# AlexGeControl/Visual-Inertial-Odometry

Measured on AMD Instinct MI355X. Metric: GN iterations/s, 11-frame (10-keyframe) window, 20k landmarks per GPU, higher is better.
Workload: dtype f64

## Files before the change

visual-inertial-odometry_amd/csrc/vio_imu_math.h:

```cpp
#ifndef VIO_IMU_MATH_H
#define VIO_IMU_MATH_H

#pragma clang fp contract(off)

#include "vio_device_math.h"
#include "vio_types.h"

#define O_P 0
#define O_R 3
#define O_V 6
#define O_BA 9
#define O_BG 12

#pragma clang fp contract(off)
__device__ __forceinline__ void nc_quat_to_R(const double *q, double *R) {
    const double x = q[0], y = q[1], z = q[2], w = q[3];
    const double tx = 2 * x, ty = 2 * y, tz = 2 * z;
    const double twx = tx * w, twy = ty * w, twz = tz * w;
    const double txx = tx * x, txy = ty * x, txz = tz * x;
    const double tyy = ty * y, tyz = tz * y, tzz = tz * z;
    R[0] = 1 - (tyy + tzz); R[1] = txy - twz;       R[2] = txz + twy;
    R[3] = txy + twz;       R[4] = 1 - (txx + tzz); R[5] = tyz - twx;
    R[6] = txz - twy;       R[7] = tyz + twx;       R[8] = 1 - (txx + tyy);
}
__device__ __forceinline__ void nc_m3_mul(const double *A, const double *B, double *C) {
#pragma unroll
    for (int i = 0; i < 3; ++i)
#pragma unroll
        for (int j = 0; j < 3; ++j)
            C[3 * i + j] = A[3 * i] * B[j] + A[3 * i + 1] * B[3 + j] + A[3 * i + 2] * B[6 + j];
}
__device__ __forceinline__ dquat nc_qmul(dquat a, dquat b) {
    dquat r;
    r.w = a.w * b.w - a.x * b.x - a.y * b.y - a.z * b.z;
    r.x = a.w * b.x + a.x * b.w + a.y * b.z - a.z * b.y;
    r.y = a.w * b.y + a.y * b.w + a.z * b.x - a.x * b.z;
    r.z = a.w * b.z + a.z * b.w + a.x * b.y - a.y * b.x;
    return r;
}
__device__ __forceinline__ dquat nc_qinv(dquat q) {
    const double n2 = q.x * q.x + q.y * q.y + q.z * q.z + q.w * q.w;
    dquat r = {0, 0, 0, 0};
    if (n2 > 0) { r.x = -q.x / n2; r.y = -q.y / n2; r.z = -q.z / n2; r.w = q.w / n2; }
    return r;
}
__device__ __forceinline__ void nc_qrot(dquat q, const double *v, double *o) {
    double ux = q.y * v[2] - q.z * v[1], uy = q.z * v[0] - q.x * v[2], uz = q.x * v[1] - q.y * v[0];
    ux += ux; uy += uy; uz += uz;
    o[0] = v[0] + q.w * ux + (q.y * uz - q.z * uy);
    o[1] = v[1] + q.w * uy + (q.z * ux - q.x * uz);
    o[2] = v[2] + q.w * uz + (q.x * uy - q.y * ux);
}
struct ImuCommon {
    dquat Qi, Qj, Qi_inv, dq, cdq;
    double sum_dt;
    double dba[3], dbg[3];
};

__device__ __forceinline__ void d_qleft_br(dquat q, double *B) {
    double v[3] = {q.x, q.y, q.z};
    d_skew(v, B);
    B[0] += q.w; B[4] += q.w; B[8] += q.w;
}
__device__ __forceinline__ void d_qright_br(dquat q, double *B) {
    double v[3] = {q.x, q.y, q.z}, S[9];
    d_skew(v, S);
#pragma unroll
    for (int k = 0; k < 9; ++k) B[k] = -S[k];
    B[0] += q.w; B[4] += q.w; B[8] += q.w;
}

__device__ void d_imu_common(const double *pre, const double *pi, const double *si, const double *pj, ImuCommon &c) {
    c.Qi = d_qload(pi); c.Qj = d_qload(pj);
    c.Qi_inv = nc_qinv(c.Qi);
    c.sum_dt = pre[PRE_SUMDT];
    c.dq.x = pre[PRE_DQ]; c.dq.y = pre[PRE_DQ + 1]; c.dq.z = pre[PRE_DQ + 2]; c.dq.w = pre[PRE_DQ + 3];
#pragma unroll
    for (int k = 0; k < 3; ++k) { c.dba[k] = si[3 + k] - pre[PRE_BA + k]; c.dbg[k] = si[6 + k] - pre[PRE_BG + k]; }
    const double *Jm = pre + PRE_JAC;
    double th[3];
#pragma unroll
    for (int i = 0; i < 3; ++i)
        th[i] = Jm[15 * (O_R + i) + O_BG] * c.dbg[0] + Jm[15 * (O_R + i) + O_BG + 1] * c.dbg[1] + Jm[15 * (O_R + i) + O_BG + 2] * c.dbg[2];
    dquat dth = {th[0] / 2.0, th[1] / 2.0, th[2] / 2.0, 1.0};
    c.cdq = nc_qmul(c.dq, dth);
}

__device__ void d_imu_residual(const double *pre, const double *G, const double *pi, const double *si, const double *pj,
                               const double *sj, const ImuCommon &c, double *res) {
    const double *Jm = pre + PRE_JAC;
    const double sum_dt = c.sum_dt;
    double cdp[3], cdv[3];
#pragma unroll
    for (int i = 0; i < 3; ++i) {
        double a = 0, b = 0, e = 0, f = 0;
#pragma unroll
        for (int j = 0; j < 3; ++j) {
            a += Jm[15 * (O_V + i) + O_BA + j] * c.dba[j];
            b += Jm[15 * (O_V + i) + O_BG + j] * c.dbg[j];
            e += Jm[15 * (O_P + i) + O_BA + j] * c.dba[j];
            f += Jm[15 * (O_P + i) + O_BG + j] * c.dbg[j];
        }
        cdv[i] = pre[PRE_DV + i] + a + b;
        cdp[i] = pre[PRE_DP + i] + e + f;
    }
    double t[3], u[3];
#pragma unroll
    for (int k = 0; k < 3; ++k) t[k] = 0.5 * G[k] * sum_dt * sum_dt + pj[k] - pi[k] - si[k] * sum_dt;
    nc_qrot(c.Qi_inv, t, u);
#pragma unroll
    for (int k = 0; k < 3; ++k) res[O_P + k] = u[k] - cdp[k];
    dquat qe = nc_qmul(nc_qinv(c.cdq), nc_qmul(c.Qi_inv, c.Qj));
    res[O_R] = 2 * qe.x; res[O_R + 1] = 2 * qe.y; res[O_R + 2] = 2 * qe.z;
#pragma unroll
    for (int k = 0; k < 3; ++k) t[k] = G[k] * sum_dt + sj[k] - si[k];
    nc_qrot(c.Qi_inv, t, u);
#pragma unroll
    for (int k = 0; k < 3; ++k) res[O_V + k] = u[k] - cdv[k];
#pragma unroll
    for (int k = 0; k < 3; ++k) { res[O_BA + k] = sj[3 + k] - si[3 + k]; res[O_BG + k] = sj[6 + k] - si[6 + k]; }
}

__device__ __forceinline__ void d_imu_rit(const ImuCommon &c, double *RiT) {
    double qi[4] = {c.Qi_inv.x, c.Qi_inv.y, c.Qi_inv.z, c.Qi_inv.w};
    nc_quat_to_R(qi, RiT);
}
__device__ void d_imu_jac_block(int blk, const double *pre, const double *G, const double *pi, const double *si,
                                const double *pj, const double *sj, const ImuCommon &c, const double *RiT, double *sJ) {
    const double *Jm = pre + PRE_JAC;
    const double sum_dt = c.sum_dt;
    double B[9];
    int r0 = 0, c0 = 0;
    switch (blk) {
    case 0: r0 = O_P; c0 = 0 + O_P;
        for (int k = 0; k < 9; ++k) B[k] = -RiT[k];
        break;
    case 1: { r0 = O_P; c0 = 0 + O_R;
        double t[3], u[3];
        for (int k = 0; k < 3; ++k) t[k] = 0.5 * G[k] * sum_dt * sum_dt + pj[k] - pi[k] - si[k] * sum_dt;
        nc_qrot(c.Qi_inv, t, u); d_skew(u, B);
        break; }
    case 2: { r0 = O_R; c0 = 0 + O_R;
        dquat a = nc_qmul(nc_qinv(c.Qj), c.Qi), b = c.cdq;
        double La[9], Rb[9], P[9];
        d_qleft_br(a, La); d_qright_br(b, Rb); nc_m3_mul(La, Rb, P);
        const double va[3] = {a.x, a.y, a.z}, vb[3] = {b.x, b.y, b.z};
        for (int i = 0; i < 3; ++i) for (int j = 0; j < 3; ++j) B[3 * i + j] = -(va[i] * (-vb[j]) + P[3 * i + j]);
        break; }
    case 3: { r0 = O_V; c0 = 0 + O_R;
        double t[3], u[3];
        for (int k = 0; k < 3; ++k) t[k] = G[k] * sum_dt + sj[k] - si[k];
        nc_qrot(c.Qi_inv, t, u); d_skew(u, B);
        break; }
    case 4: r0 = O_P; c0 = 6 + 0;
        for (int k = 0; k < 9; ++k) B[k] = -RiT[k] * sum_dt;
        break;
    case 5: r0 = O_P; c0 = 6 + 3;
        for (int i = 0; i < 3; ++i) for (int j = 0; j < 3; ++j) B[3 * i + j] = -Jm[15 * (O_P + i) + O_BA + j];
        break;
    case 6: r0 = O_P; c0 = 6 + 6;
        for (int i = 0; i < 3; ++i) for (int j = 0; j < 3; ++j) B[3 * i + j] = -Jm[15 * (O_P + i) + O_BG + j];
        break;
    case 7: { r0 = O_R; c0 = 6 + 6;
        double L[9], nL[9], D[9];
        d_qleft_br(nc_qmul(nc_qmul(nc_qinv(c.Qj), c.Qi), c.dq), L);
        for (int k = 0; k < 9; ++k) nL[k] = -L[k];
        for (int i = 0; i < 3; ++i) for (int j = 0; j < 3; ++j) D[3 * i + j] = Jm[15 * (O_R + i) + O_BG + j];
        nc_m3_mul(nL, D, B);
        break; }
    case 8: r0 = O_V; c0 = 6 + 0;
        for (int k = 0; k < 9; ++k) B[k] = -RiT[k];
        break;
    case 9: r0 = O_V; c0 = 6 + 3;
        for (int i = 0; i < 3; ++i) for (int j = 0; j < 3; ++j) B[3 * i + j] = -Jm[15 * (O_V + i) + O_BA + j];
        break;
    case 10: r0 = O_V; c0 = 6 + 6;
        for (int i = 0; i < 3; ++i) for (int j = 0; j < 3; ++j) B[3 * i + j] = -Jm[15 * (O_V + i) + O_BG + j];
        break;
    case 11: r0 = O_P; c0 = 15 + O_P;
        for (int k = 0; k < 9; ++k) B[k] = RiT[k];
        break;
    case 12: { r0 = O_R; c0 = 15 + O_R;
        d_qleft_br(nc_qmul(nc_qmul(nc_qinv(c.cdq), c.Qi_inv), c.Qj), B);
        break; }
    case 13: r0 = O_V; c0 = 21 + 0;
        for (int k = 0; k < 9; ++k) B[k] = RiT[k];
        break;
    default: return;
    }
    for (int i = 0; i < 3; ++i) for (int j = 0; j < 3; ++j) sJ[30 * (r0 + i) + c0 + j] = B[3 * i + j];
}

#pragma clang fp contract(fast)

#endif
```

visual-inertial-odometry_amd/csrc/vio_pose_solve_chain.h:

```cpp
#ifndef VIO_POSE_SOLVE_CHAIN_H
#define VIO_POSE_SOLVE_CHAIN_H

#define CH_NS 11
#define CH_TS 11
#define CH_SCSZ (16 * CH_TS)
#define CH_S9SZ (9 * CH_TS)
#define CH_OFF_SC 0
#define CH_OFF_SO (CH_OFF_SC + CH_NS * 5 * CH_SCSZ)
#define CH_OFF_SD (CH_OFF_SO + 10 * CH_S9SZ)
#define CH_OFF_CC (CH_OFF_SD + CH_NS * CH_S9SZ)
#define CH_OFF_Y (CH_OFF_CC + 15 * PS_TS)
#define CH_YC 176
#define CH_NDIM 256
#define CH_PACKED ((CH_OFF_Y + CH_NDIM + 1) & ~1)
#define CH_SET_STRIDE 16128
#define CH_OFF_SM CH_PACKED
#define CH_OFF_MC (CH_OFF_SM + CH_NS * CH_S9SZ)
#define CH_OFF_D (CH_OFF_MC + PS_TS)
#define CH_OFF_X (CH_OFF_D + CH_NDIM)
#define CH_OFF_I9 (CH_OFF_X + CH_NDIM)
#define CH_OFF_I16 (CH_OFF_I9 + CH_S9SZ)
#define CH_OFF_NZ (CH_OFF_I16 + PS_TS)
#define CH_LDS_CORE (CH_OFF_NZ + 32)
static_assert(CH_NS * CH_S9SZ >= CH_NS * 64, "the back-substitution's scratch (11 x 64) lives in the SD tiles");
// ... 370 lines not shown
#pragma unroll
                for (int k = 0; k < 3; ++k) if (lane + 64 * k < STATE_STRIDE) sState[lane + 64 * k] = st[k];
                if (test_here) {
                    double w[3];
#pragma unroll
                    for (int k = 0; k < 3; ++k) w[k] = d_wave_sum_to_lane63(er[k] * er[k]);
                    const int valid = d_imu_mask(T);
                    double t_imu = 0.0;
#pragma unroll
                    for (int k = 0; k < 10; ++k) { const double c = d_readlane(ichi, k); if ((valid >> k) & 1) t_imu += c; }
                    if (lane == 63) {
                        double total = tv[0] + t_imu;
                        if (T.has_prior) total += sqrt((w[0] + w[1]) + w[2]);
                        const double tempChi = 0.5 * total;
                        const double scale = 0.5 * (tv[1] + ((tv[3] + tv[4]) + tv[5])) + 1e-6;
                        lm->chi_try = tempChi;
                        lm->scale = scale;
                        lm->rho = (tv[2] - tempChi) / scale;
                        lm->trials += 1;
                        lm->chi = tempChi;
                        lm->cur = cur;
                        lm->accepted = 1;
                        lm->naccepted += 1;
                        lm->need_linearize = 1;
                        lm->false_cnt = 0;
                        if (!isfinite(tempChi)) lm->finite = 0;
                    }
                }
            }
        }
    } else {
    if (SPLIT) {
        xs0 = cfi[CH_OFF_SM + tid];
        if (tid < CH_NS * CH_S9SZ - PS_THREADS) xs1 = cfi[CH_OFF_SM + PS_THREADS + tid];
        if (tid < CH_YC) { xd = cfi[CH_OFF_D + tid]; xy = cfi[CH_OFF_Y + tid]; }
        if (tid < 2) xe = cfi[CH_OFF_NZ + tid];
    }
    for (int pass = 0; pass < 2; ++pass) {
        const double2 *src = reinterpret_cast<const double2 *>(T.Pg + set * CH_SET_STRIDE);
        const double2 *csrc = reinterpret_cast<const double2 *>(cfi);
        double2 *dst = reinterpret_cast<double2 *>(P);
        static_assert((CH_PACKED / 2 + PS_THREADS - 1) / PS_THREADS == 8, "copy below is written for 8 rounds");
        static_assert(CH_OFF_SD % 2 == 0, "the range that comes from cfi is whole double2s");
#define CH_FROM_CFI(i2) (SPLIT && (i2) < CH_OFF_SD / 2)
#define CH_LD(q) const double2 v##q = (CH_FROM_CFI(tid + q * PS_THREADS) ? csrc : src)[min(tid + q * PS_THREADS, CH_PACKED / 2 - 1)];
#define CH_ST(q) dst[min(tid + q * PS_THREADS, CH_PACKED / 2 - 1)] = v##q;
        CH_LD(0) CH_LD(1) CH_LD(2) CH_LD(3) CH_LD(4) CH_LD(5) CH_LD(6) CH_LD(7)
        if (pass == 0) {
            double stv = (tid < STATE_STRIDE) ? T.state[cur * STATE_STRIDE + tid] : 0.0;
            const double stv1 = (lm_loop && tid < STATE_STRIDE) ? T.state[STATE_STRIDE + tid] : 0.0;
            const bool test_here = d_step_owed(T, VIO_GN_TEST_PREV);
            double t_chi = 0.0, t_step = 0.0, t_lmchi = 0.0, t_imu = 0.0, t_sp = 0.0;
            if (test_here) {
                const int lc = lm_loop ? (lm->cur ^ lm->pending) : cur;
                double e2 = 0.0;
                if (T.has_prior && tid < VIO_PRD) { const double er = T.errprior[lc * VIO_PRD_PAD + tid]; e2 = er * er; }
                if (tid < 192) { const double w = d_wave_sum_to_lane63(e2); if (lane == 63) sB[tid >> 6] = w; }
                if (uwave == 0) {
                    const int valid = d_imu_mask(T);
                    const double ichi = T.imu_out[min(lane, 9) * IMU_OUT + IMU_CHI];
                    t_chi = T.vis[VIS_CHI]; t_step = T.vis[VIS_STEP + 1]; t_lmchi = lm->chi;
                    t_sp = (T.sp_part[0] + T.sp_part[1]) + T.sp_part[2];
#pragma unroll
                    for (int k = 0; k < 10; ++k) { const double c = d_readlane(ichi, k); if ((valid >> k) & 1) t_imu += c; }
                }
            }
            int pend0 = 0, sys0 = 0;
            if (lm_loop && tid == 0 && test_here) { d_lm_load(lm, sLm); pend0 = lm->pending; sys0 = lm->sys; }
            if (lm_loop && tid == 0 && !test_here) {
                int go = 1, rej = 0, sys = lm->sys;
                d_lm_load(lm, sLm);
                if (lm->pending) {
                    d_lm_verdict(sLm, lm, 0, lm->chi_try, lm->scale, sLm.cur);
                    if (sLm.accepted) sys ^= 1; else rej = 1;
                    go = !sLm.stop;
                }
                sX[0] = go ? 1.0 : 0.0; sX[1] = (double)sLm.cur; sX[2] = sLm.lambda; sX[3] = (double)sys; sX[4] = (double)rej;
            }
            CH_ST(0) CH_ST(1) CH_ST(2) CH_ST(3) CH_ST(4) CH_ST(5) CH_ST(6) CH_ST(7)
            __syncthreads();
            if (test_here) {
                if (tid == 0) {
                    double total = t_chi + t_imu;
                    if (T.has_prior) total += sqrt((sB[0] + sB[1]) + sB[2]);
                    const double tempChi = 0.5 * total;
                    const double scale = 0.5 * (t_step + t_sp) + 1e-6;
                    lm->chi_try = tempChi;
                    lm->scale = scale;
                    if (!lm_loop) {
                        lm->rho = (t_lmchi - tempChi) / scale;
                        lm->trials += 1;
                        lm->chi = tempChi;
                        lm->cur = cur;
                        lm->accepted = 1;
                        lm->naccepted += 1;
                        lm->need_linearize = 1;
                        lm->false_cnt = 0;
                        if (!isfinite(tempChi)) lm->finite = 0;
                    } else {
                        int go = 1, rej = 0, sys = sys0;
                        if (pend0) {
                            d_lm_verdict(sLm, lm, 0, tempChi, scale, sLm.cur);
                            if (sLm.accepted) sys ^= 1; else rej = 1;
                            go = !sLm.stop;
                        }
                        sX[0] = go ? 1.0 : 0.0; sX[1] = (double)sLm.cur; sX[2] = sLm.lambda; sX[3] = (double)sys; sX[4] = (double)rej;
                    }
                }
                if (lm_loop) __syncthreads();
            }
            int set_now = 0;
            if (lm_loop) {
                if (tid == 0) { d_lm_store(lm, sLm); lm->sys = (int)sX[3]; lm->pending = sX[0] != 0.0 ? 1 : 0; }
                if (sX[0] == 0.0) return;
                cur = (int)sX[1]; lambda = sX[2]; set_now = (int)sX[3];
                if (cur) stv = stv1;
            }
            if (tid < STATE_STRIDE) sState[tid] = stv;
            if (set_now == set) break;
            set = set_now;
            __syncthreads();
        } else {
            CH_ST(0) CH_ST(1) CH_ST(2) CH_ST(3) CH_ST(4) CH_ST(5) CH_ST(6) CH_ST(7)
            __syncthreads();
        }
#undef CH_LD
#undef CH_ST
#undef CH_FROM_CFI
    }
    if (tid < n) {
        const int d = ch_dim(tid);
        if (d >= CH_YC) P[ch_cc_elem(d - CH_YC, d - CH_YC)] += lambda;
        else if (!SPLIT) P[ch_sd(d >> 4) + (d & 15) * (CH_TS + 1)] += lambda;
    } else if (tid < n + 8) {
        P[ch_cc_elem(72 + tid - n, 72 + tid - n)] = 1.0;
    } else if (tid >= 256 && tid < 256 + CH_S9SZ + PS_TS) {
        const int i = tid - 256;
        P[CH_OFF_I9 + i] = (i < CH_S9SZ) ? ((i / CH_TS == i % CH_TS) ? 1.0 : 0.0) : (((i - CH_S9SZ) / PS_TROW == (i - CH_S9SZ) % PS_TROW) ? 1.0 : 0.0);
    } else if (tid >= 640 && tid < 640 + CH_NDIM) {
        if (!SPLIT || tid - 640 >= CH_YC) P[CH_OFF_D + tid - 640] = 1.0;
    }
    if (SPLIT) {
        P[CH_OFF_SM + tid] = xs0;
        if (tid < CH_NS * CH_S9SZ - PS_THREADS) P[CH_OFF_SM + PS_THREADS + tid] = xs1;
        if (tid < CH_YC) { P[CH_OFF_D + tid] = xd; P[CH_OFF_Y + tid] = xy; }
        if (tid < 2) P[CH_OFF_NZ + tid] = xe;
    } else {
        for (int i = tid; i < CH_NS * CH_S9SZ; i += PS_THREADS) P[CH_OFF_SM + i] = 0.0;
    }
    __syncthreads();
    }
    CH_OUT(0);
    const int trial = cur ^ 1;
    const bool prior_here = T.has_prior && !(T.gn_flags & VIO_GN_PRIOR_LATER);
    const int lm_dim = T.lm_dim;
    double *pairtab_trial = T.pairtab + trial * PAIRTAB_STRIDE;
    double *pw = P + CH_OFF_CC;
    auto mid1 = [&](int ln) {
        if (prior_here || CH_DIAG_SKIP == 2) return;
        if (ln < 12) {
            const double *p = (ln == 0) ? sState + STATE_EXT : sState + STATE_POSE + 7 * (ln - 1);
            const double *d = (ln == 0) ? sX + CH_YC + 66 : sX + CH_YC + 6 * (ln - 1);
            double dd[6], tmp[7];
#pragma unroll
            for (int k = 0; k < 6; ++k) dd[k] = d[k];
            d_pose_plus(p, dd, tmp);
            double *q = (ln == 0) ? pw + STATE_EXT : pw + STATE_POSE + 7 * (ln - 1);
#pragma unroll
            for (int k = 0; k < 7; ++k) q[k] = tmp[k];
        }
        __builtin_amdgcn_wave_barrier();
        asm volatile("" ::: "memory");
        if (lm_dim != 3) d_pair_rotations(pw, pw + 96, ln);
    };
    auto mid2 = [&](int idx, int ln) {
        if (prior_here || lm_dim == 3 || CH_DIAG_SKIP == 1 || CH_DIAG_SKIP == 2) return;
        d_pair_rows(pw, pairtab_trial, pw + 96, ln + 64 * idx, 14 * 64);
    };
    const bool ext_trivial = T.ext_fixed && !T.marg_mode;
    if (SPLIT) {
        unsigned long long t0__ = 0ull;
#ifdef VIO_STAMPS
        t0__ = __builtin_amdgcn_s_memtime();
        if (tid == 0) { g_ch_dbg = T.dbg; g_ch_t0 = t0__; }
#endif
        const unsigned lo = (unsigned)P[CH_OFF_NZ], hi = (unsigned)P[CH_OFF_NZ + 1];
        const unsigned long long eff = ((unsigned long long)__builtin_amdgcn_readfirstlane(hi) << 32) | (unsigned long long)(unsigned)__builtin_amdgcn_readfirstlane(lo);
        ch_camera_solve<true>(P, tid, ch_lane(lane), eff, mid1, mid2, T.dbg, t0__, ext_trivial);
    } else {
        ch_factor_solve(P, tid, mid1, mid2, T.dbg, ext_trivial, early);
    }
    CH_OUT(2);
    for (int i = tid; i < n; i += PS_THREADS) sDx[i] = sX[ch_dim(i)];
    if (tid >= 192 && tid < 384 && T.sp_part) {
        const int i = tid - 192;
        const double dxi = (i < n) ? sX[ch_dim(min(i, n - 1))] : 0.0;
        const double bi = early ? bf_early : ((i < n) ? T.bfull[set * VIO_PD_PAD + i] : 0.0);
        const double w = d_wave_sum_to_lane63((i < n) ? dxi * (lambda * dxi + bi) : 0.0);
        if (lane == 63) T.sp_part[i >> 6] = w;
    }
    if (!prior_here) {
        if (tid >= 128 && tid < 128 + 84) sState[tid - 128] = P[CH_OFF_CC + tid - 128];
        else if (tid >= 256 && tid < 256 + 99) { const int e = tid - 256; sState[STATE_SB + e] += sX[(e / 9) * 16 + (e % 9 < 3 ? 6 + e % 9 : (e % 9 < 6 ? e % 9 : e % 9 - 6))]; }
        d_lds_barrier();
        if (tid >= 192 && tid < 192 + n) T.dx[tid - 192] = sDx[tid - 192];
        if (tid >= 384 && tid < 384 + STATE_STRIDE) T.state[trial * STATE_STRIDE + (tid - 384)] = sState[tid - 384];
        CH_OUT(3);
        return;
    }
    __syncthreads();

    if (uwave < 2) {
        if (tid < 12) {
            double *p = (tid == 0) ? sState + STATE_EXT : sState + STATE_POSE + 7 * (tid - 1);
            const double *d = (tid == 0) ? sDx : sDx + 6 + 15 * (tid - 1);
            double tmp[7];
            d_pose_plus(p, d, tmp);
            for (int k = 0; k < 7; ++k) p[k] = tmp[k];
        } else if (tid >= 16 && tid < 16 + 99) {
            const int e = tid - 16, f = e / 9, k = e % 9;
            sState[STATE_SB + e] = sState[STATE_SB + e] + sDx[12 + 15 * f + k];
        }
        __syncthreads();
        if (T.lm_dim != 3) d_pair_rotations(sState, sR, tid);
        __syncthreads();
    } else {
        {
            double hp[PS_PRIOR_ROWS][3], bp[PS_PRIOR_ROWS];
#pragma unroll
            for (int r = 0; r < PS_PRIOR_ROWS; ++r) {
                const int i = (uwave - 2) + 14 * r;
#pragma unroll
                for (int q = 0; q < 3; ++q) {
                    const int j = lane + 64 * q;
                    hp[r][q] = (i < n && j < n) ? T.Hprior[i * n + j] : 0.0;
                }
                bp[r] = (i < n) ? T.bprior[cur * VIO_PD_PAD + i] : 0.0;
            }
            const double x0 = sDx[lane], x1 = sDx[lane + 64], x2 = (lane + 128 < n) ? sDx[lane + 128] : 0.0;
#pragma unroll
            for (int r = 0; r < PS_PRIOR_ROWS; ++r) {
                const int i = (uwave - 2) + 14 * r;
                const double v = d_bprior_dot(hp[r][0], hp[r][1], hp[r][2], x0, x1, x2, bp[r]);
                if (lane == 63 && i < n) { sB[i] = v; T.bprior[trial * VIO_PD_PAD + i] = v; }
            }
        }
        __syncthreads();
        double jp[PS_JT_ROWS][3];
#pragma unroll
        for (int r = 0; r < PS_JT_ROWS; ++r) {
            const int i = (uwave - 2) + 14 * r;
#pragma unroll
            for (int q = 0; q < 3; ++q) {
                const int j = lane + 64 * q;
                jp[r][q] = (i < VIO_PRD && j < VIO_PRD) ? T.Jtinv[i * VIO_PRD + j] : 0.0;
            }
        }
        __syncthreads();
        {
            const double y0 = sB[lane], y1 = sB[lane + 64], y2 = (lane + 128 < VIO_PRD) ? sB[lane + 128] : 0.0;
#pragma unroll
            for (int r = 0; r < PS_JT_ROWS; ++r) {
                const int i = (uwave - 2) + 14 * r;
                const double s = d_errprior_dot(jp[r][0], jp[r][1], jp[r][2], y0, y1, y2);
                if (lane == 63 && i < VIO_PRD) T.errprior[trial * VIO_PRD_PAD + i] = s;
            }
        }
    }
    if (T.lm_dim != 3) d_pair_rows(sState, T.pairtab + trial * PAIRTAB_STRIDE, sR, tid, PS_THREADS);
    if (tid >= 192 && tid < 192 + n) T.dx[tid - 192] = sDx[tid - 192];
    if (tid >= 384 && tid < 384 + STATE_STRIDE) T.state[trial * STATE_STRIDE + (tid - 384)] = sState[tid - 384];
    CH_OUT(3);
}
__global__ __launch_bounds__(PS_THREADS) void k_pose_solve_c(DeviceTables T) { d_pose_solve_chain_body<false>(T); }
__global__ __launch_bounds__(PS_THREADS) void k_pose_solve_cb(BatchArgs a) { const DeviceTables T = d_batch_tables(a); d_pose_solve_chain_body<false>(T); }
__global__ __launch_bounds__(PS_THREADS) void k_pose_solve_cs(DeviceTables T) { d_pose_solve_chain_body<true>(T); }

__device__ __forceinline__ void ch_chain_pre_store(const double *P, int tid, unsigned long long eff, double *cfi) {
    {
        const double2 *s2 = reinterpret_cast<const double2 *>(P);
        double2 *d2 = reinterpret_cast<double2 *>(cfi);
        constexpr int N2 = CH_OFF_SD / 2;
        static_assert(5 * PS_THREADS < N2 && N2 <= 6 * PS_THREADS, "six rounds");
        const double2 v0 = s2[tid], v1 = s2[tid + PS_THREADS], v2 = s2[tid + 2 * PS_THREADS], v3 = s2[tid + 3 * PS_THREADS], v4 = s2[tid + 4 * PS_THREADS];
        const int i5 = tid + 5 * PS_THREADS;
        double2 v5 = make_double2(0.0, 0.0);
        if (i5 < N2) v5 = s2[i5];
        d2[tid] = v0; d2[tid + PS_THREADS] = v1; d2[tid + 2 * PS_THREADS] = v2; d2[tid + 3 * PS_THREADS] = v3; d2[tid + 4 * PS_THREADS] = v4;
        if (i5 < N2) d2[i5] = v5;
    }
    for (int i = tid; i < CH_NS * CH_S9SZ; i += PS_THREADS) cfi[CH_OFF_SM + i] = P[CH_OFF_SM + i];
    if (tid < CH_YC) { cfi[CH_OFF_D + tid] = P[CH_OFF_D + tid]; cfi[CH_OFF_Y + tid] = P[CH_OFF_Y + tid]; }
    if (tid == 0) { cfi[CH_OFF_NZ] = (double)(unsigned)(eff & 0xffffffffull); cfi[CH_OFF_NZ + 1] = (double)(unsigned)(eff >> 32); }
}
__device__ __forceinline__ void ch_chain_pre_init(double *P, int tid) {
    if (tid >= 256 && tid < 256 + CH_S9SZ) { const int i = tid - 256; P[CH_OFF_I9 + i] = (i / CH_TS == i % CH_TS) ? 1.0 : 0.0; }
    else if (tid >= 640 && tid < 640 + CH_YC) P[CH_OFF_D + tid - 640] = 1.0;
    for (int i = tid; i < CH_NS * CH_S9SZ; i += PS_THREADS) P[CH_OFF_SM + i] = 0.0;
}
#define CPI_PRE 0
#define CPI_J (CPI_PRE + 10 * PRE_STRIDE)
#define CPI_ST (CPI_J + 10 * 450)
#define CPI_CM (CPI_ST + 184)
#define CPI_JTI(k) ((k) < 9 ? CH_OFF_CC + 450 * (k) : CH_LDS_CORE)
#define CPI_VEC (CH_LDS_CORE + 450)
#define CPI_BP (CPI_VEC + 640)
#define CPI_PN (CPI_BP + VIO_PD_PAD)
#define CPI_END (CPI_PN + 2)
#define CPI_NTILES (55 + 10 + 11)
#define CPI_FLAGS (CPI_NTILES + 99)
static_assert(CPI_CM + 400 <= CH_OFF_CC && CH_OFF_CC + 9 * 450 <= CH_OFF_Y, "staging fits the image's place");
static_assert(sizeof(ImuCommon) == 27 * 8, "ImuCommon is staged as 27 doubles");
__host__ __device__ inline int cpi_vb(int cg) { return cg < 2 ? 0 : (cg < 5 ? 1 : (cg < 7 ? 2 : 3)); }
__host__ __device__ inline void cpi_tile(int tau, int &ca, int &cb) {
    if (tau < 20) { ca = tau / 10; cb = tau % 10; }
    else if (tau < 44) { const int q = tau - 20; ca = 2 + q / 8; cb = 2 + q % 8; }
    else if (tau < 54) { const int q = tau - 44; ca = 5 + q / 5; cb = 5 + q % 5; }
    else { const int q = tau - 54; ca = 7 + q / 3; cb = 7 + q % 3; }
}
__device__ __forceinline__ int cpi_tau(int ca, int cb) { return ca < 2 ? ca * 10 + cb : (ca < 5 ? 20 + (ca - 2) * 8 + (cb - 2) : (ca < 7 ? 44 + (ca - 5) * 5 + (cb - 5) : 54 + (ca - 7) * 3 + (cb - 7))); }
__device__ __forceinline__ unsigned cpi_rows(int cg) {
    return cg == 0 ? 0x01u : cg == 1 ? 0x07u : cg == 2 ? 0x05u : cg == 3 ? 0x0du : cg == 4 ? 0x17u : cg == 5 ? 0x01u : cg == 6 ? 0x02u : cg == 7 ? 0x04u : cg == 8 ? 0x08u : 0x10u;
}
__host__ __device__ inline int cpi_tile_of(int p) { return p < CH_OFF_SO ? p / CH_SCSZ : (p < CH_OFF_SD ? 55 + (p - CH_OFF_SO) / CH_S9SZ : 65 + (p - CH_OFF_SD) / CH_S9SZ); }
__host__ __device__ inline int cpi_tile_base(int t) { return t < 55 ? t * CH_SCSZ : (t < 65 ? CH_OFF_SO + (t - 55) * CH_S9SZ : CH_OFF_SD + (t - 65) * CH_S9SZ); }
__host__ __device__ inline int cpi_tile_size(int t) { return t < 55 ? CH_SCSZ : CH_S9SZ; }

__device__ __forceinline__ void d_chain_pre_item(const DeviceTables &T) {
    double *P = dyn_smem;
    const int tid = threadIdx.x, lane = tid & 63;
    const int wave = __builtin_amdgcn_readfirstlane(tid >> 6);
    const int cur = d_cur(T);
    const int valid = d_imu_mask(T);
    const bool owe_prior = d_step_owed(T, VIO_GN_BACKSUB_PREV) && T.has_prior;
    const double lambda = T.lm->lambda;
#ifdef VIO_STAMPS
    unsigned long long *cdbg = T.dbg ? T.dbg + 16 * (size_t)(T.n_items + 11) : nullptr;
    const unsigned long long cp_t0 = __builtin_amdgcn_s_memtime();
#define CP_STAMP(i) do { if (tid == 0 && cdbg) cdbg[i] = __builtin_amdgcn_s_memtime() - cp_t0; } while (0)
#else
    unsigned long long *cdbg = nullptr;
    const unsigned long long cp_t0 = 0ull;
#define CP_STAMP(i) do { } while (0)
#endif
    {
        double pv[5];
#pragma unroll
        for (int q = 0; q < 5; ++q) { const int i = tid + q * PS_THREADS; pv[q] = i < 10 * PRE_STRIDE ? T.pre[i] : 0.0; }
        const double sv = tid < STATE_STRIDE ? T.state[cur * STATE_STRIDE + tid] : 0.0;
        int pn = 0, pm = 0, prow = -1;
        double bpv = 0.0;
        bool bp_skip = false;
        if (T.has_prior) {
            pn = T.prior_list[0]; pm = T.prior_list[1];
            if (tid >= 128 && tid < 128 + 99) {
                const int r = tid - 128;
                bpv = T.bprior[(owe_prior ? cur ^ 1 : cur) * VIO_PD_PAD + 12 + 15 * (r / 9) + r % 9];
                bp_skip = owe_prior && T.prior_flags[CPI_NTILES + r] != 0;
            }
            if (owe_prior && wave < 15) prow = T.prior_list[2 + min(wave, 98)];
        }
        if (wave == 15 && lane < 10 && ((valid >> lane) & 1)) {
            const int k = lane;
            const double *pre = T.pre + k * PRE_STRIDE, *st = T.state + cur * STATE_STRIDE;
            ImuCommon c;
            double RiT[9];
            d_imu_common(pre, st + STATE_POSE + 7 * k, st + STATE_SB + 9 * k, st + STATE_POSE + 7 * k + 7, c);
            d_imu_rit(c, RiT);
            double *cm = P + CPI_CM + 40 * k;
            const double *cc = reinterpret_cast<const double *>(&c);
#pragma unroll
            for (int q = 0; q < 27; ++q) cm[q] = cc[q];
#pragma unroll
            for (int q = 0; q < 9; ++q) cm[28 + q] = RiT[q];
        }
#pragma unroll
        for (int q = 0; q < 5; ++q) { const int i = tid + q * PS_THREADS; if (i < 10 * PRE_STRIDE) P[CPI_PRE + i] = pv[q]; }
        if (tid < STATE_STRIDE) P[CPI_ST + tid] = sv;
        double2 *zj = reinterpret_cast<double2 *>(P + CPI_J);
        static_assert(CPI_J % 2 == 0, "J is zeroed as double2");
        for (int i = tid; i < 10 * 450 / 2; i += PS_THREADS) zj[i] = make_double2(0.0, 0.0);
        if (tid < CH_YC) P[CH_OFF_Y + tid] = 0.0;
        ch_chain_pre_init(P, tid);
        if (T.has_prior && tid >= 128 && tid < 128 + 99 && !bp_skip) { const int r = tid - 128; P[CPI_BP + 12 + 15 * (r / 9) + r % 9] = bpv; }
        if (owe_prior && wave < 15 && wave < pm) {
            const bool in2 = lane + 128 < VIO_PD;
            const double x0 = T.dx[lane], x1 = T.dx[lane + 64], x2 = in2 ? T.dx[lane + 128] : 0.0;
            for (int q = wave; q < pm; q += 15) {
                const int r = q == wave ? prow : T.prior_list[2 + q];
                const int i = 12 + 15 * (r / 9) + r % 9;
                const double *hr = T.Hprior + (size_t)i * VIO_PD;
                const double v = d_bprior_dot(hr[lane], hr[lane + 64], in2 ? hr[lane + 128] : 0.0, x0, x1, x2, T.bprior[(cur ^ 1) * VIO_PD_PAD + i]);
                if (lane == 63) P[CPI_BP + i] = v;
            }
        }
        if (tid == 0) { reinterpret_cast<int *>(P + CPI_PN)[0] = pn; reinterpret_cast<int *>(P + CPI_PN)[1] = pm; }
    }
    CP_STAMP(0);
    __syncthreads();
    CP_STAMP(1);
    const int task = __builtin_amdgcn_readfirstlane((int)((0xfa85d964b310c72eull >> (4 * wave)) & 15ull));
    if (lane < 10 && ((valid >> lane) & 1)) {
        const int k = lane;
        const double *pre = P + CPI_PRE + k * PRE_STRIDE, *st = P + CPI_ST;
        const double *pi = st + STATE_POSE + 7 * k, *pj = pi + 7, *si = st + STATE_SB + 9 * k, *sj = si + 9;
        double *sJ = P + CPI_J + 450 * k, *sr = P + CPI_VEC + 64 * k;
        const double *cm = P + CPI_CM + 40 * k;
        if (task < 15) {
            const ImuCommon &c = *reinterpret_cast<const ImuCommon *>(cm);
            if (task < 14) {
                d_imu_jac_block(task, pre, T.gravity, pi, si, pj, sj, c, cm + 28, sJ);
            } else {
                double r[15];
                d_imu_residual(pre, T.gravity, pi, si, pj, sj, c, r);
                for (int i = 0; i < 15; ++i) sr[i] = r[i];
            }
        } else {
            for (int i = 0; i < 3; ++i) {
                sJ[30 * (O_BA + i) + 6 + 3 + i] = -1.0; sJ[30 * (O_BG + i) + 6 + 6 + i] = -1.0;
                sJ[30 * (O_BA + i) + 21 + 3 + i] = 1.0; sJ[30 * (O_BG + i) + 21 + 6 + i] = 1.0;
            }
        }
    }
    CP_STAMP(2);
#ifdef VIO_STAMPS
    if (lane == 0 && cdbg) cdbg[32 + wave] = __builtin_amdgcn_s_memtime() - cp_t0;
#endif
    __syncthreads();
    CP_STAMP(3);
    if (wave < 10) {
        const int ca = wave, k = lane / 5, j0 = 3 * (lane % 5);
        if (lane < 50 && ((valid >> k) & 1)) {
            const double *sJ = P + CPI_J + 450 * k + 3 * ca, *sI = P + CPI_PRE + k * PRE_STRIDE + PRE_INFO + j0;
            double acc[3][3] = {{0.0, 0.0, 0.0}, {0.0, 0.0, 0.0}, {0.0, 0.0, 0.0}};
            const unsigned rows = cpi_rows(ca);
#pragma unroll
            for (int rb = 0; rb < 5; ++rb) {
                if (!((rows >> rb) & 1)) continue;
                double ja[3][3], ib[3][3];
#pragma unroll
                for (int ii = 0; ii < 3; ++ii)
#pragma unroll
                    for (int u = 0; u < 3; ++u) { ja[ii][u] = sJ[30 * (3 * rb + ii) + u]; ib[ii][u] = sI[15 * (3 * rb + ii) + u]; }
#pragma unroll
                for (int ii = 0; ii < 3; ++ii)
#pragma unroll
                    for (int u = 0; u < 3; ++u)
#pragma unroll
                        for (int v = 0; v < 3; ++v) acc[u][v] = fma(ja[ii][u], ib[ii][v], acc[u][v]);
            }
            double *o = P + CPI_JTI(k) + 15 * 3 * ca + j0;
#pragma unroll
            for (int u = 0; u < 3; ++u)
#pragma unroll
                for (int v = 0; v < 3; ++v) o[15 * u + v] = acc[u][v];
        }
    } else if (wave < 13) {
        const int t = (wave - 10) * 64 + lane;
        const int k = t / 15, i = t % 15;
        if (t < 150 && ((valid >> k) & 1)) {
            const double *sI = P + CPI_PRE + k * PRE_STRIDE + PRE_INFO, *sr = P + CPI_VEC + 64 * k;
            double sum = 0;
            for (int j = 0; j < 15; ++j) sum = fma(sI[15 * i + j], sr[j], sum);
            P[CPI_VEC + 64 * k + 16 + i] = sum;
        }
    }
    CP_STAMP(4);
    __syncthreads();
    CP_STAMP(5);
    double tv[9];
    unsigned tmap[9];
    int t_edge = -1;
#pragma unroll
    for (int q = 0; q < 9; ++q) { tv[q] = 0.0; tmap[q] = 0xffff0000u | (unsigned)CH_OFF_X; }
    if (wave < 15) {
        const int cb = wave < 5 ? wave : 5 + (wave - 5) / 2;
        const int nca = cb < 2 ? 2 : (cb < 5 ? 5 : (cb < 7 ? 7 : 10));
        const int ntask = 10 * nca, half = (ntask + 1) / 2;
        const int q0 = wave < 5 ? 0 : ((wave - 5) & 1) * half, q1 = wave < 5 ? ntask : (((wave - 5) & 1) ? ntask : half);
        const int q = q0 + lane;
        const int k = q / nca, ca = q % nca;
        if (q < q1 && ((valid >> k) & 1)) {
            t_edge = k;
            const int tau = cpi_tau(ca, cb);
#pragma unroll
            for (int e = 0; e < 9; ++e) tmap[e] = T.imu_map[(k * 63 + tau) * 9 + e];
            const double *sA = P + CPI_JTI(k) + 15 * 3 * ca, *sJ = P + CPI_J + 450 * k + 3 * cb;
            double acc[3][3] = {{0.0, 0.0, 0.0}, {0.0, 0.0, 0.0}, {0.0, 0.0, 0.0}};
            const unsigned rows = cpi_rows(cb);
#pragma unroll
            for (int rb = 0; rb < 5; ++rb) {
                if (!((rows >> rb) & 1)) continue;
                double aa[3][3], jb[3][3];
#pragma unroll
                for (int jj = 0; jj < 3; ++jj)
#pragma unroll
                    for (int u = 0; u < 3; ++u) { aa[jj][u] = sA[15 * u + 3 * rb + jj]; jb[jj][u] = sJ[30 * (3 * rb + jj) + u]; }
#pragma unroll
                for (int jj = 0; jj < 3; ++jj)
#pragma unroll
                    for (int u = 0; u < 3; ++u)
#pragma unroll
                        for (int v = 0; v < 3; ++v) acc[u][v] = fma(aa[jj][u], jb[jj][v], acc[u][v]);
            }
            double *out = T.imu_out + k * IMU_OUT + IMU_T + 30 * 3 * ca + 3 * cb;
#pragma unroll
            for (int u = 0; u < 3; ++u)
#pragma unroll
                for (int v = 0; v < 3; ++v) { tv[3 * u + v] = acc[u][v]; out[30 * u + v] = acc[u][v]; }
        }
    }
    if (wave < 15 && lane < 20) {
        const int t = wave * 20 + lane;
        const int k = t / 30, a = t % 30;
        if ((valid >> k) & 1) {
            const double *sJ = P + CPI_J + 450 * k + a, *sIr = P + CPI_VEC + 64 * k + 16;
            double ja[15], ir[15];
#pragma unroll
            for (int i = 0; i < 15; ++i) { ja[i] = sJ[30 * i]; ir[i] = sIr[i]; }
            double sum = 0;
#pragma unroll
            for (int i = 0; i < 15; ++i) sum = fma(ja[i], ir[i], sum);
            P[CPI_VEC + 64 * k + 32 + a] = sum;
            T.imu_out[k * IMU_OUT + IMU_G + a] = sum;
        }
    } else if (wave == 15 && lane < 10) {
        const int k = lane;
        if ((valid >> k) & 1) {
            const double *sr = P + CPI_VEC + 64 * k, *sIr = sr + 16;
            double sum = 0;
            for (int i = 0; i < 15; ++i) sum = fma(sr[i], sIr[i], sum);
            T.imu_out[k * IMU_OUT + IMU_CHI] = sum;
        }
    }
    double pr[2] = {0.0, 0.0};
    int pr_pos[2] = {-1, -1};
    const int pn = T.has_prior ? reinterpret_cast<const int *>(P + CPI_PN)[0] : 0;
    if (pn <= 2 * PS_THREADS) {
#pragma unroll
        for (int h = 0; h < 2; ++h) if (tid + h * PS_THREADS < pn) { pr_pos[h] = T.prior_list[128 + tid + h * PS_THREADS]; pr[h] = T.prior_cval[tid + h * PS_THREADS]; }
    }
    CP_STAMP(6);
#ifdef VIO_STAMPS
    if (lane == 0 && cdbg) cdbg[48 + wave] = __builtin_amdgcn_s_memtime() - cp_t0;
#endif
    __syncthreads();
    CP_STAMP(7);
    {
        double2 *z = reinterpret_cast<double2 *>(P);
        for (int i = tid; i < (CH_OFF_CC + 1) / 2; i += PS_THREADS) z[i] = make_double2(0.0, 0.0);
    }
    __syncthreads();
    CP_STAMP(8);
    bool has_mirror = false;
#pragma unroll
    for (int q = 0; q < 9; ++q) has_mirror = has_mirror || (tmap[q] >> 16) != 0xffffu;
    has_mirror = has_mirror && t_edge >= 0;
    const bool wave_mirror = __ballot(has_mirror) != 0ull;
    if (t_edge >= 0 && (t_edge & 1) == 0) {
#pragma unroll
        for (int q = 0; q < 9; ++q) P[tmap[q] & 0xffffu] = tv[q];
        if (wave_mirror) {
#pragma unroll
            for (int q = 0; q < 9; ++q) if ((tmap[q] >> 16) != 0xffffu) P[tmap[q] >> 16] = tv[q];
        }
    }
    CP_STAMP(14);
    __syncthreads();
    CP_STAMP(15);
    if (t_edge >= 0 && (t_edge & 1) == 1) {
        double old[9];
#pragma unroll
        for (int q = 0; q < 9; ++q) old[q] = P[tmap[q] & 0xffffu];
#pragma unroll
        for (int q = 0; q < 9; ++q) P[tmap[q] & 0xffffu] = old[q] + tv[q];
        if (wave_mirror) {
#pragma unroll
            for (int q = 0; q < 9; ++q) if ((tmap[q] >> 16) != 0xffffu) P[tmap[q] >> 16] = old[q] + tv[q];
        }
    }
    __syncthreads();
    CP_STAMP(9);
    if (T.has_prior) {
        if (pn > 2 * PS_THREADS) { for (int i = tid; i < CH_OFF_CC; i += PS_THREADS) P[i] += T.prior_simg[i]; }
        else {
            if (pr_pos[0] >= 0) P[pr_pos[0]] += pr[0];
            if (pr_pos[1] >= 0) P[pr_pos[1]] += pr[1];
        }
    }
    if (tid < 99) {
        const int f = tid / 9, i = 12 + 15 * f + tid % 9;
        double extra = 0.0;
        for (int k = f - 1; k <= f; ++k) {
            if (k < 0 || k >= 10 || !((valid >> k) & 1)) continue;
            const int a = i - (6 + 15 * k);
            extra -= P[CPI_VEC + 64 * k + 32 + a];
        }
        if (T.has_prior) extra += P[CPI_BP + i];
        P[CH_OFF_Y + ch_dim(i)] = extra;
    }
    __syncthreads();
    CP_STAMP(10);
    if (tid < CH_NS * 9) { const int e = tid / 9, k = tid % 9; P[ch_sd(e) + k * (CH_TS + 1)] += lambda; }
    __syncthreads();
    CP_STAMP(11);
    const unsigned long long eff = ch_chain_elimination<false>(P, tid, ch_lane(lane), cdbg, cp_t0);
    CP_STAMP(12);
    ch_chain_pre_store(P, tid, eff, T.cfi);
    CP_STAMP(13);
#undef CP_STAMP
}

__global__ __launch_bounds__(192) void k_prior_simg(DeviceTables T) {
    const int r = blockIdx.x, t = threadIdx.x;
    if (r >= 99 || t >= VIO_PD) return;
    const int i = 12 + 15 * (r / 9) + r % 9;
    if (T.Hprior[i * VIO_PD + t] != 0.0) T.prior_flags[CPI_NTILES + r] = 1;
    if (!(full_to_cam(t) >= 0 || t <= i)) return;
    const int I = max(i, t), J = min(i, t);
    const bool mask = T.ext_fixed && !T.marg_mode && (I < 6 || J < 6);
    const double v = mask ? 0.0 : T.Hprior[I * VIO_PD + J];
    int p1, p2;
    ch_entry_pos(I, J, p1, p2);
    if (p1 >= 0) { T.prior_simg[p1] = v; if (v != 0.0) T.prior_flags[cpi_tile_of(p1)] = 1; }
    if (p2 >= 0) T.prior_simg[p2] = v;
}

__global__ __launch_bounds__(PS_THREADS) void k_prior_compact(DeviceTables T) {
    __shared__ int sCnt[PS_THREADS + 1];
    const int tid = threadIdx.x;
    constexpr int PER = (CH_OFF_CC + PS_THREADS - 1) / PS_THREADS;
    int c = 0;
    for (int q = 0; q < PER; ++q) { const int p = tid * PER + q; if (p < CH_OFF_CC && T.prior_simg[p] != 0.0) ++c; }
    sCnt[tid + 1] = c;
    if (tid == 0) sCnt[0] = 0;
    __syncthreads();
    if (tid == 0) for (int i = 1; i <= PS_THREADS; ++i) sCnt[i] += sCnt[i - 1];
    __syncthreads();
    int o = sCnt[tid];
    for (int q = 0; q < PER; ++q) {
        const int p = tid * PER + q;
        if (p < CH_OFF_CC) { const double v = T.prior_simg[p]; if (v != 0.0) { T.prior_list[128 + o] = p; T.prior_cval[o] = v; ++o; } }
    }
    if (tid == 0) {
        T.prior_list[0] = sCnt[PS_THREADS];
        int m = 0;
        for (int r = 0; r < 99; ++r) if (T.prior_flags[CPI_NTILES + r]) T.prior_list[2 + m++] = r;
        T.prior_list[1] = m;
    }
}

__global__ __launch_bounds__(PS_THREADS) void k_chain_pre(DeviceTables T) {
    double *P = dyn_smem;
    const int tid = threadIdx.x;
    const double lambda = T.lm->lambda;
    const double *img = T.Pg + d_set_w(T) * CH_SET_STRIDE;
    for (int i = tid; i < CH_OFF_CC; i += PS_THREADS) P[i] = img[i];
    if (tid < CH_YC) P[CH_OFF_Y + tid] = img[CH_OFF_Y + tid];
    ch_chain_pre_init(P, tid);
    __syncthreads();
    if (tid < CH_NS * 9) { const int e = tid / 9, k = tid % 9; P[ch_sd(e) + k * (CH_TS + 1)] += lambda; }
    __syncthreads();
    const unsigned long long eff = ch_chain_elimination<false>(P, tid, ch_lane(tid & 63), T.dbg, 0ull);
    ch_chain_pre_store(P, tid, eff, T.cfi);
}

#ifdef VIO_DEBUG_ENTRY_POINTS
__global__ __launch_bounds__(PS_THREADS) void k_chain_solve_test(const double *img, double lambda, double *x_nat, double *lds_dump) {
    double *P = dyn_smem;
    const int tid = threadIdx.x;
    for (int i = tid; i < CH_PACKED; i += PS_THREADS) P[i] = img[i];
    for (int i = CH_PACKED + tid; i < CH_LDS_CORE; i += PS_THREADS) P[i] = 0.0;
    __syncthreads();
    if (tid < PS_N) {
        const int d = ch_dim(tid);
        if (d >= CH_YC) P[ch_cc_elem(d - CH_YC, d - CH_YC)] += lambda;
        else P[ch_sd(d >> 4) + (d & 15) * (CH_TS + 1)] += lambda;
    } else if (tid < PS_N + 8) {
        P[ch_cc_elem(72 + tid - PS_N, 72 + tid - PS_N)] = 1.0;
    } else if (tid >= 256 && tid < 256 + CH_S9SZ + PS_TS) {
        const int i = tid - 256;
        P[CH_OFF_I9 + i] = (i < CH_S9SZ) ? ((i / CH_TS == i % CH_TS) ? 1.0 : 0.0) : (((i - CH_S9SZ) / PS_TROW == (i - CH_S9SZ) % PS_TROW) ? 1.0 : 0.0);
    } else if (tid >= 640 && tid < 640 + CH_NDIM) {
        P[CH_OFF_D + tid - 640] = 1.0;
    }
    for (int i = tid; i < CH_NS * CH_S9SZ; i += PS_THREADS) P[CH_OFF_SM + i] = 0.0;
    __syncthreads();
    ch_factor_solve(P, tid, [](int) {}, [](int, int) {});
    if (tid < PS_N) x_nat[tid] = P[CH_OFF_X + ch_dim(tid)];
    if (lds_dump) for (int i = tid; i < CH_LDS_CORE; i += PS_THREADS) lds_dump[i] = P[i];
}
#endif
#endif
#endif
```

Baseline: 20580.

## Rebalance IMU wave tasks and spread LDS zeroing across earlier phases

New measurement: 20580. About the same (-0.0%).

```diff
diff --git a/visual-inertial-odometry_amd/csrc/vio_imu_math.h b/visual-inertial-odometry_amd/csrc/vio_imu_math.h
--- a/visual-inertial-odometry_amd/csrc/vio_imu_math.h
+++ b/visual-inertial-odometry_amd/csrc/vio_imu_math.h
@@ -121,6 +121,53 @@
     for (int k = 0; k < 3; ++k) { res[O_BA + k] = sj[3 + k] - si[3 + k]; res[O_BG + k] = sj[6 + k] - si[6 + k]; }
 }
 
+__device__ __forceinline__ void d_imu_residual_part(int part, const double *pre, const double *G, const double *pi, const double *si, const double *pj,
+                                                    const double *sj, const ImuCommon &c, double *res) {
+    const double *Jm = pre + PRE_JAC;
+    const double sum_dt = c.sum_dt;
+    double t[3], u[3];
+    if (part == 0) {
+        double cdp[3];
+#pragma unroll
+        for (int i = 0; i < 3; ++i) {
+            double e = 0, f = 0;
+#pragma unroll
+            for (int j = 0; j < 3; ++j) {
+                e += Jm[15 * (O_P + i) + O_BA + j] * c.dba[j];
+                f += Jm[15 * (O_P + i) + O_BG + j] * c.dbg[j];
+            }
+            cdp[i] = pre[PRE_DP + i] + e + f;
+        }
+#pragma unroll
+        for (int k = 0; k < 3; ++k) t[k] = 0.5 * G[k] * sum_dt * sum_dt + pj[k] - pi[k] - si[k] * sum_dt;
+        nc_qrot(c.Qi_inv, t, u);
+#pragma unroll
+        for (int k = 0; k < 3; ++k) res[O_P + k] = u[k] - cdp[k];
+    } else if (part == 1) {
+        dquat qe = nc_qmul(nc_qinv(c.cdq), nc_qmul(c.Qi_inv, c.Qj));
+        res[O_R] = 2 * qe.x; res[O_R + 1] = 2 * qe.y; res[O_R + 2] = 2 * qe.z;
+    } else {
+        double cdv[3];
+#pragma unroll
+        for (int i = 0; i < 3; ++i) {
+            double a = 0, b = 0;
+#pragma unroll
+            for (int j = 0; j < 3; ++j) {
+                a += Jm[15 * (O_V + i) + O_BA + j] * c.dba[j];
+                b += Jm[15 * (O_V + i) + O_BG + j] * c.dbg[j];
+            }
+            cdv[i] = pre[PRE_DV + i] + a + b;
+        }
+#pragma unroll
+        for (int k = 0; k < 3; ++k) t[k] = G[k] * sum_dt + sj[k] - si[k];
+        nc_qrot(c.Qi_inv, t, u);
+#pragma unroll
+        for (int k = 0; k < 3; ++k) res[O_V + k] = u[k] - cdv[k];
+#pragma unroll
+        for (int k = 0; k < 3; ++k) { res[O_BA + k] = sj[3 + k] - si[3 + k]; res[O_BG + k] = sj[6 + k] - si[6 + k]; }
+    }
+}
+
 __device__ __forceinline__ void d_imu_rit(const ImuCommon &c, double *RiT) {
     double qi[4] = {c.Qi_inv.x, c.Qi_inv.y, c.Qi_inv.z, c.Qi_inv.w};
     nc_quat_to_R(qi, RiT);
diff --git a/visual-inertial-odometry_amd/csrc/vio_pose_solve_chain.h b/visual-inertial-odometry_amd/csrc/vio_pose_solve_chain.h
--- a/visual-inertial-odometry_amd/csrc/vio_pose_solve_chain.h
+++ b/visual-inertial-odometry_amd/csrc/vio_pose_solve_chain.h
@@ -696,6 +696,7 @@
 #define CPI_J (CPI_PRE + 10 * PRE_STRIDE)
 #define CPI_ST (CPI_J + 10 * 450)
 #define CPI_CM (CPI_ST + 184)
+#define CPI_ZTAIL (CPI_CM + 400)
 #define CPI_JTI(k) ((k) < 9 ? CH_OFF_CC + 450 * (k) : CH_LDS_CORE)
 #define CPI_VEC (CH_LDS_CORE + 450)
 #define CPI_BP (CPI_VEC + 640)
@@ -768,14 +769,17 @@
 #pragma unroll
             for (int q = 0; q < 9; ++q) cm[28 + q] = RiT[q];
         }
+        if (wave < 15) {
+            double2 *zj = reinterpret_cast<double2 *>(P + CPI_J);
+            static_assert(CPI_J % 2 == 0, "J is zeroed as double2");
+            for (int i = tid; i < 10 * 450 / 2; i += PS_THREADS - 64) zj[i] = make_double2(0.0, 0.0);
+            for (int i = CPI_ZTAIL + tid; i < CH_OFF_CC; i += PS_THREADS - 64) P[i] = 0.0;
+        }
+        if (tid < CH_YC) P[CH_OFF_Y + tid] = 0.0;
+        ch_chain_pre_init(P, tid);
 #pragma unroll
         for (int q = 0; q < 5; ++q) { const int i = tid + q * PS_THREADS; if (i < 10 * PRE_STRIDE) P[CPI_PRE + i] = pv[q]; }
         if (tid < STATE_STRIDE) P[CPI_ST + tid] = sv;
-        double2 *zj = reinterpret_cast<double2 *>(P + CPI_J);
-        static_assert(CPI_J % 2 == 0, "J is zeroed as double2");
-        for (int i = tid; i < 10 * 450 / 2; i += PS_THREADS) zj[i] = make_double2(0.0, 0.0);
-        if (tid < CH_YC) P[CH_OFF_Y + tid] = 0.0;
-        ch_chain_pre_init(P, tid);
         if (T.has_prior && tid >= 128 && tid < 128 + 99 && !bp_skip) { const int r = tid - 128; P[CPI_BP + 12 + 15 * (r / 9) + r % 9] = bpv; }
         if (owe_prior && wave < 15 && wave < pm) {
             const bool in2 = lane + 128 < VIO_PD;
@@ -793,21 +797,21 @@
     CP_STAMP(0);
     __syncthreads();
     CP_STAMP(1);
-    const int task = __builtin_amdgcn_readfirstlane((int)((0xfa85d964b310c72eull >> (4 * wave)) & 15ull));
+    const int task = __builtin_amdgcn_readfirstlane((int)((0xea965480f3f1c72full >> (4 * wave)) & 15ull));
+    const int task2 = wave == 8 ? 11 : (wave == 9 ? 13 : -1);
     if (lane < 10 && ((valid >> lane) & 1)) {
         const int k = lane;
         const double *pre = P + CPI_PRE + k * PRE_STRIDE, *st = P + CPI_ST;
         const double *pi = st + STATE_POSE + 7 * k, *pj = pi + 7, *si = st + STATE_SB + 9 * k, *sj = si + 9;
         double *sJ = P + CPI_J + 450 * k, *sr = P + CPI_VEC + 64 * k;
         const double *cm = P + CPI_CM + 40 * k;
-        if (task < 15) {
+        if (task != 14) {
             const ImuCommon &c = *reinterpret_cast<const ImuCommon *>(cm);
             if (task < 14) {
                 d_imu_jac_block(task, pre, T.gravity, pi, si, pj, sj, c, cm + 28, sJ);
+                if (task2 >= 0) d_imu_jac_block(task2, pre, T.gravity, pi, si, pj, sj, c, cm + 28, sJ);
             } else {
-                double r[15];
-                d_imu_residual(pre, T.gravity, pi, si, pj, sj, c, r);
-                for (int i = 0; i < 15; ++i) sr[i] = r[i];
+                d_imu_residual_part(wave == 0 ? 0 : (wave == 5 ? 1 : 2), pre, T.gravity, pi, si, pj, sj, c, sr);
             }
         } else {
             for (int i = 0; i < 3; ++i) {
@@ -854,14 +858,24 @@
         const int k = t / 15, i = t % 15;
         if (t < 150 && ((valid >> k) & 1)) {
             const double *sI = P + CPI_PRE + k * PRE_STRIDE + PRE_INFO, *sr = P + CPI_VEC + 64 * k;
+            double ia[15], ra[15];
+#pragma unroll
+            for (int j = 0; j < 15; ++j) { ia[j] = sI[15 * i + j]; ra[j] = sr[j]; }
             double sum = 0;
-            for (int j = 0; j < 15; ++j) sum = fma(sI[15 * i + j], sr[j], sum);
+#pragma unroll
+            for (int j = 0; j < 15; ++j) sum = fma(ia[j], ra[j], sum);
             P[CPI_VEC + 64 * k + 16 + i] = sum;
         }
     }
     CP_STAMP(4);
     __syncthreads();
     CP_STAMP(5);
+    {
+        static_assert(CPI_PRE == 0 && CPI_J % 2 == 0 && CPI_ST % 2 == 0 && CPI_ZTAIL % 2 == 0, "zeroed as double2");
+        double2 *z = reinterpret_cast<double2 *>(P);
+        for (int i = tid; i < CPI_J / 2; i += PS_THREADS) z[i] = make_double2(0.0, 0.0);
+        for (int i = CPI_ST / 2 + tid; i < CPI_ZTAIL / 2; i += PS_THREADS) z[i] = make_double2(0.0, 0.0);
+    }
     double tv[9];
     unsigned tmap[9];
     int t_edge = -1;
@@ -898,12 +912,18 @@
                         for (int v = 0; v < 3; ++v) acc[u][v] = fma(aa[jj][u], jb[jj][v], acc[u][v]);
             }
             double *out = T.imu_out + k * IMU_OUT + IMU_T + 30 * 3 * ca + 3 * cb;
+#ifdef VIO_STAMPS
+            if (lane == 0 && cdbg) cdbg[118 + wave] = __builtin_amdgcn_s_memtime() - cp_t0;
+#endif
 #pragma unroll
             for (int u = 0; u < 3; ++u)
 #pragma unroll
                 for (int v = 0; v < 3; ++v) { tv[3 * u + v] = acc[u][v]; out[30 * u + v] = acc[u][v]; }
         }
     }
+#ifdef VIO_STAMPS
+    if (lane == 0 && cdbg) cdbg[96 + wave] = __builtin_amdgcn_s_memtime() - cp_t0;
+#endif
     if (wave < 15 && lane < 20) {
         const int t = wave * 20 + lane;
         const int k = t / 30, a = t % 30;
@@ -922,8 +942,12 @@
         const int k = lane;
         if ((valid >> k) & 1) {
             const double *sr = P + CPI_VEC + 64 * k, *sIr = sr + 16;
+            double ra[15], ia[15];
+#pragma unroll
+            for (int i = 0; i < 15; ++i) { ra[i] = sr[i]; ia[i] = sIr[i]; }
             double sum = 0;
-            for (int i = 0; i < 15; ++i) sum = fma(sr[i], sIr[i], sum);
+#pragma unroll
+            for (int i = 0; i < 15; ++i) sum = fma(ra[i], ia[i], sum);
             T.imu_out[k * IMU_OUT + IMU_CHI] = sum;
         }
     }
@@ -942,7 +966,7 @@
     CP_STAMP(7);
     {
         double2 *z = reinterpret_cast<double2 *>(P);
-        for (int i = tid; i < (CH_OFF_CC + 1) / 2; i += PS_THREADS) z[i] = make_double2(0.0, 0.0);
+        for (int i = CPI_J / 2 + tid; i < CPI_ST / 2; i += PS_THREADS) z[i] = make_double2(0.0, 0.0);
     }
     __syncthreads();
     CP_STAMP(8);
```
